# jbirky/alabi

Measured on AMD Instinct MI355X. Metric: surrogate_mcmc_samples_per_sec, higher is better.
Workload: dtype f64

## Files before the change

alabi_amd/_lib.py:

```python
from __future__ import annotations

import ctypes as C
import os
import subprocess

_HERE = os.path.dirname(os.path.abspath(__file__))
CSRC = os.path.join(_HERE, "csrc")
LIB_PATH = os.path.join(CSRC, "libalabi_hip.so")

OK, NOT_PD, BAD_ARG, HIP_ERROR, NOT_COMPUTED, TIMEOUT = 0, 1, 2, 3, 4, 5
UTILITY_CODES = {"bape": 0, "agp": 1, "jones": 2}
KERNEL_CODES = {"ExpSquaredKernel": 0, "Matern32Kernel": 1, "Matern52Kernel": 2, "RationalQuadraticKernel": 3}
MAX_DIM = 64

_vp, _i, _ll, _d = C.c_void_p, C.c_int, C.c_longlong, C.c_double
_ull = C.c_ulonglong
_pd = C.POINTER(C.c_double)
_pi = C.POINTER(C.c_int)
_pll = C.POINTER(C.c_longlong)

SIGNATURES = {
    "alabi_abi_version": (_i, []),
    "alabi_status_string": (C.c_char_p, [_i]),
    "alabi_last_error": (C.c_char_p, []),
# ... 29 lines not shown
    "alabi_kernel_matrix": (_i, [_vp, _i, _vp, _i, _i, _i, _d, _d, _pd, _vp, _vp]),
    "alabi_utility_scan": (_i, [_vp, _i, _vp, _ll, _pd, _d, _vp, _vp, _vp, _pd, _pll, _vp]),
    "alabi_utility_polish": (_i, [_vp, _i, _vp, _vp, _d, _i, _vp, _pd, _pi, _vp]),
    "alabi_utility_eval": (_i, [_i, _vp, _ll, _i, _pd, _d, _vp, _vp, _vp, _vp]),
    "alabi_ens_create": (_i, [_vp, _i, _i, _i, _pd, _ull, C.POINTER(_vp)]),
    "alabi_ens_destroy": (_i, [_vp]),
    "alabi_ens_set_logp_affine": (_i, [_vp, _d, _d]),
    "alabi_ens_set_normal_prior": (_i, [_vp, _pd, _pd]),
    "alabi_ens_set_logp_map": (_i, [_vp, _i]),
    "alabi_ens_surrogate": (_i, [_vp, _vp, _i, _vp, _vp]),
    "alabi_ens_propose": (_i, [_vp, _vp, _i, _i, _i, _vp, _vp, _vp]),
    "alabi_ens_accept": (_i, [_vp, _vp, _vp, _i, _i, _vp, _vp, _vp, _vp]),
    "alabi_ens_set_moves": (_i, [_vp, _i, _pi, _pd, _pd, _pd]),
    "alabi_ens_set_stream": (_i, [_vp, _i]),
    "alabi_ens_last_path": (_i, [_vp, _pi]),
    "alabi_ens_group_plan": (_i, [_vp, _pi]),
    "alabi_ens_lnprob": (_i, [_vp, _vp, _vp, _vp]),
    "alabi_ens_run": (_i, [_vp, _vp, _vp, _ll, _ll, _i, _d, _vp, _vp, _vp, _vp]),
    "alabi_chain_autocorr": (_i, [_vp, _ll, _i, _i, _vp, _vp]),
    "alabi_ens_draw": (_i, [_vp, _ll, _i, _d, _vp]),
    "alabi_ens_half_step": (_i, [_vp, _vp, _vp, _i, _i, _i, _i, _vp, _vp]),
    "alabi_dist_unique_id": (_i, [_vp]),
    "alabi_dist_comm_create": (_i, [_vp, _i, _i, C.POINTER(_vp)]),
    "alabi_dist_comm_create_callback": (_i, [_vp, _vp, _i, _i, C.POINTER(_vp)]),
    "alabi_dist_comm_destroy": (_i, [_vp]),
    "alabi_dist_comm_stats": (_i, [_vp, _pll]),
    "alabi_ens_run_sharded": (_i, [_vp, _vp, _vp, _vp, _ll, _ll, _i, _d, _vp, _vp, _vp, _vp]),
    "alabi_ens_step_lists": (_i, [_vp, _i, _vp, _pi, _vp]),
    "alabi_ens_step_with_randoms": (_i, [_vp, _vp, _vp, _vp, _i, _vp, _vp, _vp, _d, _vp, _vp]),
    "alabi_ens_export_draws": (_i, [_vp, _ll, _d, _vp, _pi, _vp, _vp, _vp, _vp, _vp, _vp]),
# ... 101 lines not shown
```

alabi_amd/csrc/api.hip:

```cpp
#include <atomic>
#include <cmath>
#include <cstdlib>
#include <mutex>
#include <new>
#include <vector>

#include "gp_device.hpp"

namespace alabi {
thread_local std::string g_last_error;

static inline hipStream_t as_stream(void* s) { return reinterpret_cast<hipStream_t>(s); }

__global__ void __launch_bounds__(256)
copy_factor_kernel(const double* __restrict__ L, int ld, int N, double* __restrict__ out) {
    size_t e = (size_t)blockIdx.x * 256 + threadIdx.x;
    if (e >= (size_t)N * N) return;
    int r = (int)(e / N), c = (int)(e % N);
    out[e] = (c <= r) ? L[(size_t)r * ld + c] : 0.0;
}

namespace {
struct CachedBuf { void* p; size_t bytes; };
std::mutex g_cache_mu;
// ... 560 lines not shown
int alabi_ens_destroy(alabi_ens* e) {
    if (!e) return ALABI_OK;
    if (e->graph_exec) (void)hipGraphExecDestroy(e->graph_exec);
    free_draws(e->draws);
    free_draws(e->draws2);
    free_move_buffers(e->mv);
    if (e->side_stream) (void)hipStreamDestroy(e->side_stream);
    if (e->ev_free) (void)hipEventDestroy(e->ev_free);
    if (e->ev_drawn) (void)hipEventDestroy(e->ev_drawn);
    if (e->run_state) (void)hipFree(e->run_state);
    if (e->consts) (void)hipFree(e->consts);
    if (e->hist) (void)hipFree(e->hist);
    if (e->part) (void)hipFree(e->part);
    if (e->cand) (void)hipFree(e->cand);
    if (e->err) (void)hipFree(e->err);
    delete e;
    return ALABI_OK;
}

int alabi_ens_set_normal_prior(alabi_ens* e, const double* mean, const double* std) {
    if (!e || !mean || !std) return ALABI_BAD_ARGUMENT;
    e->has_prior = 0; e->prior_const = 0.0;
    for (int k = 0; k < ALABI_MAX_DIM; ++k) { e->prior_mean[k] = 0.0; e->prior_istd[k] = 0.0; }
    for (int k = 0; k < e->d; ++k) {
        if (std::isfinite(mean[k]) && std::isfinite(std[k]) && std[k] > 0.0) {
            e->prior_mean[k] = mean[k];
            e->prior_istd[k] = 1.0 / std[k];
            e->prior_const += -std::log(std[k]) - 0.9189385332046727;
            e->has_prior = 1;
        }
// ... 38 lines not shown
    if (n > 0) { const int st = ensure_move_buffers(e); if (st != ALABI_OK) return st; }
    mt.n = n;
    e->moves = mt;
    e->has_de = de;
    e->drawn_n = 0;
    e->settings_gen++;
    if (e->graph_exec) { (void)hipGraphExecDestroy(e->graph_exec); e->graph_exec = nullptr; }
    return ALABI_OK;
}

int alabi_ens_set_stream(alabi_ens* e, int enabled) {
    if (!e) return ALABI_BAD_ARGUMENT;
    if (enabled && !(e->hist && e->err)) return ALABI_BAD_ARGUMENT;
    e->stream_ok = enabled ? 1 : 0;
    e->settings_gen++;
    return ALABI_OK;
}

int alabi_ens_last_path(alabi_ens* e, int* path) {
    if (!e || !path) return ALABI_BAD_ARGUMENT;
    *path = e->last_path;
    return ALABI_OK;
}

int alabi_ens_group_plan(alabi_ens* e, int* out) {
    if (!e || !out) return ALABI_BAD_ARGUMENT;
    for (int i = 0; i < 8; ++i) out[i] = e->group_plan[i];
    return ALABI_OK;
}

// ... 80 lines not shown
    hipStream_t s = as_stream(stream);
    int st;
    if ((st = sync_consts(e, s)) != ALABI_OK) return st;
    e->last_path = 0;
    const char* genv = getenv("ALABI_ENS_GROUP");
    const bool group_off = genv && genv[0] == '0', group_pref = genv && genv[0] == '1';
    const bool can_stream = ens_stream_fits(e);
    const bool crowded = can_stream && e->stream_grid > 0 && ((e->W + 1) / 2 + e->stream_grid - 1) / e->stream_grid >= 4;
    const bool use_group = !e->has_de && e->stream_ok && s != nullptr && !group_off && (group_pref || !can_stream || crowded) && ens_group_fits(e) &&
                           ens_group_buffers(e, s);
    if (!e->has_de && e->stream_ok && s != nullptr && (can_stream || use_group)) {
        e->last_path = use_group ? 3 : 1;
        const int need = (int)(nsteps < e->chunk_cap ? nsteps : e->chunk_cap);
        const int clean_rows = e->hist_clean;
        e->hist_clean = 0;
        if (use_group && (st = set_run_state(e, step0, 0, s)) != ALABI_OK) return st;
        ALABI_HIP_CHECK(hipMemsetAsync(e->err, 0, sizeof(int), s));
        long long remaining = nsteps;
        const bool two_sets = !use_group && nsteps > e->chunk_cap && ens_draw_ahead_ready(e);
        bool ahead_issued = false;
        while (remaining > 0) {
            const int K = (int)(remaining < e->chunk_cap ? remaining : e->chunk_cap);
            const long long done = nsteps - remaining;
            if (use_group) {
                if ((st = launch_ens_draw(e, K, a, s)) != ALABI_OK) return st;
                if ((st = launch_ens_group(e, coords, logp, K, thin_by, chain, chain_logp, n_accept, s)) != ALABI_OK) return st;
                if ((st = launch_ens_advance(e, K, s)) != ALABI_OK) return st;
            } else {
                const bool odd = two_sets && ((done / e->chunk_cap) & 1);
                const bool ahead = two_sets && remaining > K;
                const DrawBuffers& cur = odd ? e->draws2 : e->draws;
                if (ahead_issued) ALABI_HIP_CHECK(hipStreamWaitEvent(s, e->ev_drawn, 0));
                else if ((st = launch_ens_draw_at(e, cur, K, a, false, step0 + done, s)) != ALABI_OK) return st;
                ahead_issued = false;
                if (ahead) ALABI_HIP_CHECK(hipEventRecord(e->ev_free, s));
                if ((st = launch_ens_stream_kernel(e, cur, coords, logp, K, done == 0, (done == 0 && clean_rows < need) ? need : 0, s)) != ALABI_OK)
                    return st;
                if (ahead) {
                    const long long rem2 = remaining - K;
                    const int K2 = (int)(rem2 < e->chunk_cap ? rem2 : e->chunk_cap);
                    ALABI_HIP_CHECK(hipStreamWaitEvent(e->side_stream, e->ev_free, 0));
                    if ((st = launch_ens_draw_at(e, odd ? e->draws : e->draws2, K2, a, false, step0 + done + K, e->side_stream)) != ALABI_OK)
                        return st;
                    ALABI_HIP_CHECK(hipEventRecord(e->ev_drawn, e->side_stream));
                    ahead_issued = true;
                }
                if ((st = launch_ens_stream_epilogue(e, coords, logp, K, thin_by, chain, chain_logp, n_accept, step0 + done + K, done, s)) != ALABI_OK)
                    return st;
            }
            remaining -= K;
        }
        int flag = 0;
        ALABI_HIP_CHECK(hipMemcpyAsync(&flag, e->err, sizeof(int), hipMemcpyDeviceToHost, s));
        ALABI_HIP_CHECK(hipStreamSynchronize(s));
        e->hist_clean = (!use_group && !flag) ? (clean_rows > need ? clean_rows : need) : 0;
        return flag ? ALABI_TIMEOUT : ALABI_OK;
    }
    if ((st = set_run_state(e, step0, 0, s)) != ALABI_OK) return st;
    HalfArgs h = base_args(e, coords, logp);
    h.chain = chain; h.chain_logp = chain_logp; h.n_accept = n_accept; h.thin_by = thin_by;

    const char* env = getenv("ALABI_ENS_GRAPH");
    const bool want_graph = (s != nullptr) && !(env && env[0] == '0');
    int gsteps = e->chunk_cap < 256 ? e->chunk_cap : 256;
    if (const char* gs = getenv("ALABI_ENS_GRAPH_STEPS")) {
        int v = atoi(gs);
        if (v > 0 && v <= e->chunk_cap) gsteps = v;
    }
    long long remaining = nsteps;
    if (want_graph && remaining >= 2LL * gsteps) {
// ... 171 lines not shown
```

alabi_amd/csrc/common.hpp:

```cpp
#pragma once
#include <hip/hip_runtime.h>
#include <cstdint>
#include <cstdio>
#include <cstring>
#include <string>
#include <vector>

#include "../../include/alabi_hip.h"
#include "chol_tasks.hpp"

#define ALABI_BLK 64

namespace alabi {

extern thread_local std::string g_last_error;

inline int hip_fail(hipError_t e, const char* what, const char* file, int line) {
    char buf[512];
    snprintf(buf, sizeof(buf), "%s failed at %s:%d: %s", what, file, line, hipGetErrorString(e));
    g_last_error = buf;
    return ALABI_HIP_ERROR;
}

#define ALABI_HIP_CHECK(expr)                                                    \
// ... 122 lines not shown
        double a;
        long long gp_gen;
    } graph_key{};
    int graph_steps = 0;
    long long* run_state = nullptr;
    unsigned long long* hist = nullptr;
    int* err = nullptr;
    alabi::DrawBuffers draws2{};
    hipStream_t side_stream = nullptr;
    hipEvent_t ev_free = nullptr, ev_drawn = nullptr;
    int draws2_state = 0;
    int hist_clean = 0;
    int stream_grid = 0;
    int last_path = 0;
    int stream_ok = 0;
    unsigned long long* part = nullptr;
    size_t part_words = 0;
    unsigned long long* cand = nullptr;
    size_t cand_words = 0;
    long long settings_gen = 0;
    long long serial = 0;
    int group_plan[8] = {0};
    alabi::MoveTable moves{};
    bool has_de = false;
    alabi::MoveBuffers mv{};
};

namespace alabi {
int launch_prepare_inputs(alabi_gp* gp, const double* X, int N, hipStream_t s);
int launch_assemble(alabi_gp* gp, hipStream_t s, int zero_ctl_ints = 0);
// ... 71 lines not shown
int launch_ens_draw_at(alabi_ens* e, const DrawBuffers& into, int nsteps, double a, bool from_state, long long step0, hipStream_t s);
int launch_ens_prep(alabi_ens* e, const int* order, int n0, const double* u_z, const int* partner,
                    const double* u_acc, double a, hipStream_t s);
int launch_ens_prep_de(alabi_ens* e, const int* order, int n0, const int* j1, const int* j2, const double* gamma,
                       const double* u_acc, hipStream_t s);
int launch_ens_half_args(alabi_ens* e, const HalfArgs& args, int nblocks, hipStream_t s);
int launch_ens_lnprob(alabi_ens* e, const double* coords, int nwalkers, double* logp, int gate_box, hipStream_t s);
int launch_ens_propose(alabi_ens* e, const HalfArgs& args, int nblocks, int gate_box, double* q, double* like, hipStream_t s);
int launch_ens_accept(alabi_ens* e, const HalfArgs& args, int count, const double* q, const double* lp_new, hipStream_t s);
int launch_ens_advance(alabi_ens* e, long long n, hipStream_t s);
int ens_sync_consts(alabi_ens* e, hipStream_t s);
int alabi_ens_half_step_hist(alabi_ens* e, const double* coords, const double* logp, int t, int split, int part_begin, int part_end,
                             const double* shist, double* out, hipStream_t s);
bool ens_stream_fits(const alabi_ens* e);
int launch_ens_stream_kernel(alabi_ens* e, const DrawBuffers& rec, double* coords, double* logp, int K, bool first, int fill_rows, hipStream_t s);
int launch_ens_stream_epilogue(alabi_ens* e, double* coords, double* logp, int K, int thin_by, double* chain, double* chain_logp,
                               long long* n_accept, long long step_next, long long done0, hipStream_t s);
bool ens_group_fits(const alabi_ens* e);
bool ens_group_buffers(alabi_ens* e, hipStream_t s);
int launch_ens_group(alabi_ens* e, double* coords, double* logp, int K, int thin_by, double* chain, double* chain_logp,
                     long long* n_accept, hipStream_t s);
int launch_ens_hist_prologue(alabi_ens* e, double* coords, double* logp, int K, bool fill, hipStream_t s);
int launch_ens_hist_epilogue(alabi_ens* e, double* coords, double* logp, int K, int thin_by, double* chain, double* chain_logp,
                             long long* n_accept, hipStream_t s);
}
```

alabi_amd/csrc/ensemble.hip:

```cpp
#include <cstdlib>
#include <vector>
#include "ens_device.hpp"

namespace alabi {

__device__ inline void store_record(const DrawBuffers& b, size_t pos, int wid, int cw, double zz, double lnfac, double lnu) {
    b.order[pos] = wid;
    b.cw[pos] = cw;
    b.zz[pos] = zz;
    b.lnfac[pos] = lnfac;
    b.lnu[pos] = lnu;
    unsigned long long* pk = b.packed + 4 * pos;
    pk[0] = (unsigned long long)(unsigned)wid | ((unsigned long long)(unsigned)cw << 32);
    pk[1] = (unsigned long long)__double_as_longlong(zz);
    pk[2] = (unsigned long long)__double_as_longlong(lnfac);
    pk[3] = (unsigned long long)__double_as_longlong(lnu);
}

__device__ inline void write_record(const DrawBuffers& b, size_t pos, int wid, int cw, double u_z, double u_acc,
                                    double a, int d) {
    const double t1 = (a - 1.0) * u_z + 1.0;
    const double zz = (t1 * t1) / a;
    store_record(b, pos, wid, cw, zz, ((double)d - 1.0) * log(zz), log(u_acc));
}
// ... 565 lines not shown
    const int w = p.rec.order[pos];
    if (w < 0) return;
    const double lpn = lp_new[i], lpo = p.logp[w];
    if (p.rec.lnfac[pos] + lpn - lpo > p.rec.lnu[pos]) {
        for (int k = 0; k < p.d; ++k) p.coords[(size_t)w * p.d + k] = q[(size_t)i * p.d + k];
        p.logp[w] = lpn;
        if (p.n_accept) p.n_accept[w] += 1;
    }
}

__global__ void ens_advance_kernel(long long* run_state, long long n) {
    if (threadIdx.x == 0 && blockIdx.x == 0) { run_state[0] += n; run_state[1] += n; }
}


#define ALABI_HIST_EMPTY 0x7FF8A1AB1D15EA5Eull

struct StreamArgs {
    unsigned long long* hist;
    int* err;
    DrawBuffers rec;
    const double* consts;
    const double* Xt;
    const double* alpha;
    const double* centre;
    int K, W, n0, d, Npad, spin_limit, has_prior;
    double amp, mean, prior_const;
    KernelFn kf;
};

__device__ inline unsigned long long ld_sc1(const unsigned long long* p) {
    return __hip_atomic_load(p, __ATOMIC_RELAXED, __HIP_MEMORY_SCOPE_AGENT);
}
__device__ inline void st_sc1(unsigned long long* p, unsigned long long v) {
    __hip_atomic_store(p, v, __ATOMIC_RELAXED, __HIP_MEMORY_SCOPE_AGENT);
}

#ifdef ALABI_STREAM_PROF
__device__ long long g_stream_prof[16];
#endif

template <int NW>
__device__ inline double wave_partials_tree(const double* s) {
    const f64x2* v = reinterpret_cast<const f64x2*>(s);
    auto pair = [&](int i) { return 2 * i < NW ? v[i].y + v[i].x : 0.0; };
    const double lo8 = (pair(3) + pair(2)) + (pair(1) + pair(0));
    if (NW <= 8) return lo8;
    const double hi8 = (pair(7) + pair(6)) + (pair(5) + pair(4));
    return hi8 + lo8;
}

template <int D, int PPT, int TMAX, bool GENERIC>
__global__ void __launch_bounds__(TMAX)
ens_stream_kernel(StreamArgs p) {
    __shared__ __attribute__((aligned(16))) double scratch[2][16];
    __shared__ unsigned long long rec_s[4][4];
    __shared__ __attribute__((aligned(16))) double qs_s[2][ALABI_MAX_DIM];
    __shared__ double consts_s[6][ALABI_MAX_DIM];
    __shared__ int abort_s;
    static_assert(D < ALABI_MAX_DIM && TMAX >= 192 && TMAX % 64 == 0, "ens_stream_kernel: shape");
    constexpr int TC = TMAX - 128, nwc = TC >> 6;
    const int tid = threadIdx.x, lane = tid & 63;
    const int wv = __builtin_amdgcn_readfirstlane(tid >> 6);
    const bool comm = wv == 0, service = wv == nwc + 1, compute = !comm && !service;
    const int b = blockIdx.x, e = blockIdx.y, E = gridDim.y;
// ... 351 lines not shown
    return ALABI_OK;
}

int launch_ens_hist_epilogue(alabi_ens* e, double* coords, double* logp, int K, int thin_by, double* chain, double* chain_logp,
                             long long* n_accept, hipStream_t s) {
    const int WT = e->W * e->E, row = e->d + 2;
    hipLaunchKernelGGL(ens_hist_copy_kernel, dim3((WT * row + 255) / 256), dim3(256), 0, s, coords, logp,
                       e->hist + (size_t)K * WT * row, WT, e->d, 0);
    if (chain || chain_logp || n_accept)
        hipLaunchKernelGGL(ens_hist_chain_kernel, dim3(2048), dim3(256), 0, s, e->hist, K, WT, e->d, thin_by, e->run_state,
                           e->err, chain, chain_logp, reinterpret_cast<unsigned long long*>(n_accept));
    ALABI_LAUNCH_CHECK();
    return ALABI_OK;
}

int launch_ens_stream_kernel(alabi_ens* e, const DrawBuffers& rec, double* coords, double* logp, int K, bool first, int fill_rows,
                             hipStream_t s) {
    alabi_gp* gp = e->gp;
    const int n0 = (e->W + 1) / 2;
    const int WT = e->W * e->E, row = e->d + 2;
    if (fill_rows > 0) hipLaunchKernelGGL(ens_hist_fill_kernel, dim3(1024), dim3(256), 0, s, e->hist + (size_t)WT * row, (size_t)fill_rows * WT * row);
    if (first) hipLaunchKernelGGL(ens_hist_copy_kernel, dim3((WT * row + 255) / 256), dim3(256), 0, s, coords, logp, e->hist, WT, e->d, 1);
    StreamArgs a{};
    a.hist = e->hist; a.err = e->err; a.rec = rec; a.consts = e->consts;
    const bool se = gp->kf.type == 0;
    a.Xt = se ? gp->Xc : gp->Xt; a.alpha = se ? gp->ens_h : gp->alpha; a.centre = gp->xa_centre;
    a.K = K; a.W = e->W; a.n0 = n0; a.d = e->d; a.Npad = gp->Npad; a.spin_limit = 1 << 20;
    if (const char* env = getenv("ALABI_ENS_SPIN_LIMIT")) { const int v = atoi(env); if (v > 0) a.spin_limit = v; }
    a.amp = e->lp_scale * exp(gp->log_amp); a.mean = fma(e->lp_scale, gp->mean, e->lp_shift); a.kf = gp->kf;
    a.has_prior = e->has_prior; a.prior_const = e->prior_const;
    const int db = dim_bucket(e->d);
    const int T = e->threads, ppt = ens_stream_ppt(e);
    e->last_path = 1;
    if (T == 256) {
        if (ppt == 1) { ALABI_STREAM_LAUNCH(1, 384); }
        else if (ppt == 2) { ALABI_STREAM_LAUNCH(2, 384); }
        else if (ppt == 3) { ALABI_STREAM_LAUNCH(3, 384); }
        else if (ppt == 4) { ALABI_STREAM_LAUNCH(4, 384); }
        else return ALABI_BAD_ARGUMENT;
    } else if (T == 512) {
        if (ppt == 1) { ALABI_STREAM_LAUNCH(1, 640); }
        else if (ppt == 2) { ALABI_STREAM_LAUNCH(2, 640); }
        else return ALABI_BAD_ARGUMENT;
    } else return ALABI_BAD_ARGUMENT;
    ALABI_LAUNCH_CHECK();
// ... 137 lines not shown
```

alabi_amd/sampler.py:

```python
from __future__ import annotations

import ctypes as C
import time

import numpy as np
import torch

from . import _lib
from .gp import HipGP, _dev, _to_dev
from .mcmc_utils import integrated_time
from .moves import parse_moves

__all__ = ["EnsembleSampler", "State"]


class State:
    def __init__(self, coords, log_prob=None):
        self.coords = coords
        self.log_prob = log_prob
        self.blobs = None
        self.random_state = None

    def __iter__(self):
        return iter((self.coords, self.log_prob, self.random_state))
# ... 268 lines not shown
                                                nsteps, thin_by, self.a, _lib.ptr(chain), _lib.ptr(chain_lp),
                                                _lib.ptr(self._naccept), C.c_void_p(self._stream.cuda_stream))

        st = _run()
        if st == _lib.TIMEOUT:
            self._stream.synchronize()
            self._coords.copy_(backup[0]); self._logp.copy_(backup[1]); self._naccept.copy_(backup[2])
            _lib.check(_lib.lib().alabi_ens_set_stream(self._ens, 0), "alabi_ens_set_stream")
            self.stream_fallbacks = getattr(self, "stream_fallbacks", 0) + 1
            st = _run()
        _lib.check(st, "alabi_ens_run")
        path = C.c_int(0)
        _lib.lib().alabi_ens_last_path(self._ens, C.byref(path))
        self.last_path = {1: "stream", 3: "group"}.get(path.value, "launch-per-half-step")
        self.last_stream_kernel = {1: "ens_stream_kernel", 3: "ens_group_kernel"}.get(path.value)
        self.group_plan = None
        if path.value == 3:
            plan = (C.c_int * 8)()
            _lib.lib().alabi_ens_group_plan(self._ens, plan)
            self.group_plan = dict(zip(("Q", "G", "NG", "RT", "tpm", "ltw", "KS", "lds_bytes"), (int(v) for v in plan)))
        self._stream.synchronize()
        torch.cuda.current_stream().wait_stream(self._stream)
        self.last_run_seconds = time.perf_counter() - t0
        self.iteration += nsteps
        self._rng_step += nsteps
        if nstore:
            self._chains.append(chain)
            self._chain_lps.append(chain_lp)
            self._thins.append(thin_by)
        return State(self._coords.cpu().numpy(), self._logp.cpu().numpy())
# ... 42 lines not shown
```

include/alabi_hip.h:

```cpp
#ifndef ALABI_HIP_H
#define ALABI_HIP_H

#ifdef __cplusplus
extern "C" {
#endif

#define ALABI_OK 0
#define ALABI_NOT_POSITIVE_DEFINITE 1
#define ALABI_BAD_ARGUMENT 2
#define ALABI_HIP_ERROR 3
#define ALABI_NOT_COMPUTED 4
#define ALABI_TIMEOUT 5

#define ALABI_UTILITY_BAPE 0
#define ALABI_UTILITY_AGP 1
#define ALABI_UTILITY_JONES 2

#define ALABI_MAX_DIM 64

typedef struct alabi_gp alabi_gp;
typedef struct alabi_ens alabi_ens;
typedef struct alabi_ns alabi_ns;
typedef struct alabi_kde alabi_kde;

// ... 67 lines not shown
                       void* stream);

int alabi_ens_create(alabi_gp* gp, int W, int d, int n_ensembles, const double* bounds,
                     unsigned long long seed, alabi_ens** out);
int alabi_ens_destroy(alabi_ens* ens);
int alabi_ens_set_normal_prior(alabi_ens* ens, const double* mean, const double* std);

int alabi_ens_set_logp_affine(alabi_ens* ens, double scale, double shift);

int alabi_ens_set_logp_map(alabi_ens* ens, int kind);

int alabi_ens_set_moves(alabi_ens* ens, int n, const int* kind, const double* cum, const double* p0, const double* p1);

int alabi_ens_set_stream(alabi_ens* ens, int enabled);
int alabi_ens_last_path(alabi_ens* ens, int* path );
int alabi_ens_group_plan(alabi_ens* ens, int* out );

int alabi_ens_lnprob(alabi_ens* ens, const double* coords, double* logp, void* stream);

int alabi_ens_surrogate(alabi_ens* ens, const double* points, int M, double* like, void* stream);

int alabi_ens_run(alabi_ens* ens, double* coords, double* logp, long long step0,
                  long long nsteps, int thin_by, double a, double* chain, double* chain_logp,
                  long long* n_accept, void* stream);

int alabi_chain_autocorr(const double* chain, long long n_t, int n_w, int n_d, double* acf_mean, void* stream);

int alabi_ens_draw(alabi_ens* ens, long long step0, int nsteps, double a, void* stream);
int alabi_ens_half_step(alabi_ens* ens, double* coords, double* logp, int t, int split,
                        int part_begin, int part_end, long long* n_accept, void* stream);
// ... 77 lines not shown
```

Before: 84.76 million.

## Add paired-block speculative stream kernel for ensemble MCMC sampling

Adds a new ens_pair_kernel variant of the persistent stream kernel in which each walker item is handled by two cooperating blocks. One block speculatively evaluates the surrogate on a proposal built from not-yet-final coordinates and publishes it to a separate proposal history buffer, which shortens the dependency chain between half-steps. The run loop selects the pair variant when the group path is not used and the extra buffers can be allocated. It saves coords, logp and accept counts first so that a timeout can roll back and re-run on the single-block path. This costs twice the blocks, extra history memory and fill traffic, and adds spin-wait and correctness risk.

```diff
diff --git a/alabi_amd/_lib.py b/alabi_amd/_lib.py
--- a/alabi_amd/_lib.py
+++ b/alabi_amd/_lib.py
@@ -67,6 +67,8 @@
     "alabi_ens_set_moves": (_i, [_vp, _i, _pi, _pd, _pd, _pd]),
     "alabi_ens_set_stream": (_i, [_vp, _i]),
     "alabi_ens_last_path": (_i, [_vp, _pi]),
+    "alabi_ens_stream_variant": (_i, [_vp, _pi]),
+    "alabi_ens_pair_stats": (_i, [_vp, _pll, _i]),
     "alabi_ens_group_plan": (_i, [_vp, _pi]),
     "alabi_ens_lnprob": (_i, [_vp, _vp, _vp, _vp]),
     "alabi_ens_run": (_i, [_vp, _vp, _vp, _ll, _ll, _i, _d, _vp, _vp, _vp, _vp]),
diff --git a/alabi_amd/csrc/api.hip b/alabi_amd/csrc/api.hip
--- a/alabi_amd/csrc/api.hip
+++ b/alabi_amd/csrc/api.hip
@@ -598,6 +598,7 @@
     if (e->part) (void)hipFree(e->part);
     if (e->cand) (void)hipFree(e->cand);
     if (e->err) (void)hipFree(e->err);
+    ens_pair_release(e);
     delete e;
     return ALABI_OK;
 }
@@ -666,6 +667,24 @@
     if (enabled && !(e->hist && e->err)) return ALABI_BAD_ARGUMENT;
     e->stream_ok = enabled ? 1 : 0;
     e->settings_gen++;
+    return ALABI_OK;
+}
+
+int alabi_ens_stream_variant(alabi_ens* e, int* variant) {
+    if (!e || !variant) return ALABI_BAD_ARGUMENT;
+    *variant = (e->last_path == 1) ? e->last_variant : 0;
+    return ALABI_OK;
+}
+
+int alabi_ens_pair_stats(alabi_ens* e, long long* out, int reset) {
+    if (!e || !out) return ALABI_BAD_ARGUMENT;
+    if (!e->pair_stats) {
+        ALABI_HIP_CHECK(hipMalloc(&e->pair_stats, 9 * sizeof(unsigned long long)));
+        ALABI_HIP_CHECK(hipMemset(e->pair_stats, 0, 9 * sizeof(unsigned long long)));
+    }
+    ALABI_HIP_CHECK(hipDeviceSynchronize());
+    ALABI_HIP_CHECK(hipMemcpy(out, e->pair_stats, 9 * sizeof(unsigned long long), hipMemcpyDeviceToHost));
+    if (reset) ALABI_HIP_CHECK(hipMemset(e->pair_stats, 0, 9 * sizeof(unsigned long long)));
     return ALABI_OK;
 }
 
@@ -776,6 +795,15 @@
         const int need = (int)(nsteps < e->chunk_cap ? nsteps : e->chunk_cap);
         const int clean_rows = e->hist_clean;
         e->hist_clean = 0;
+        const bool use_pair = !use_group && can_stream && ens_pair_ready(e);
+        e->last_variant = use_pair ? 1 : 0;
+        const size_t WTs = (size_t)e->W * e->E;
+        if (use_pair) {
+            double* sv = e->pair_save;
+            ALABI_HIP_CHECK(hipMemcpyAsync(sv, coords, WTs * e->d * sizeof(double), hipMemcpyDeviceToDevice, s));
+            ALABI_HIP_CHECK(hipMemcpyAsync(sv + WTs * e->d, logp, WTs * sizeof(double), hipMemcpyDeviceToDevice, s));
+            if (n_accept) ALABI_HIP_CHECK(hipMemcpyAsync(sv + WTs * (e->d + 1), n_accept, WTs * sizeof(long long), hipMemcpyDeviceToDevice, s));
+        }
         if (use_group && (st = set_run_state(e, step0, 0, s)) != ALABI_OK) return st;
         ALABI_HIP_CHECK(hipMemsetAsync(e->err, 0, sizeof(int), s));
         long long remaining = nsteps;
@@ -796,7 +824,9 @@
                 else if ((st = launch_ens_draw_at(e, cur, K, a, false, step0 + done, s)) != ALABI_OK) return st;
                 ahead_issued = false;
                 if (ahead) ALABI_HIP_CHECK(hipEventRecord(e->ev_free, s));
-                if ((st = launch_ens_stream_kernel(e, cur, coords, logp, K, done == 0, (done == 0 && clean_rows < need) ? need : 0, s)) != ALABI_OK)
+                const int fill_rows = (done == 0 && clean_rows < need) ? need : 0;
+                if ((st = use_pair ? launch_ens_pair_kernel(e, cur, coords, logp, K, done == 0, fill_rows, s)
+                                   : launch_ens_stream_kernel(e, cur, coords, logp, K, done == 0, fill_rows, s)) != ALABI_OK)
                     return st;
                 if (ahead) {
                     const long long rem2 = remaining - K;
@@ -816,6 +846,14 @@
         ALABI_HIP_CHECK(hipMemcpyAsync(&flag, e->err, sizeof(int), hipMemcpyDeviceToHost, s));
         ALABI_HIP_CHECK(hipStreamSynchronize(s));
         e->hist_clean = (!use_group && !flag) ? (clean_rows > need ? clean_rows : need) : 0;
+        if (flag && use_pair) {
+            const double* sv = e->pair_save;
+            ALABI_HIP_CHECK(hipMemcpyAsync(coords, sv, WTs * e->d * sizeof(double), hipMemcpyDeviceToDevice, s));
+            ALABI_HIP_CHECK(hipMemcpyAsync(logp, sv + WTs * e->d, WTs * sizeof(double), hipMemcpyDeviceToDevice, s));
+            if (n_accept) ALABI_HIP_CHECK(hipMemcpyAsync(n_accept, sv + WTs * (e->d + 1), WTs * sizeof(long long), hipMemcpyDeviceToDevice, s));
+            e->pair_state = -1;
+            return alabi_ens_run(e, coords, logp, step0, nsteps, thin_by, a, chain, chain_logp, n_accept, stream);
+        }
         return flag ? ALABI_TIMEOUT : ALABI_OK;
     }
     if ((st = set_run_state(e, step0, 0, s)) != ALABI_OK) return st;
diff --git a/alabi_amd/csrc/common.hpp b/alabi_amd/csrc/common.hpp
--- a/alabi_amd/csrc/common.hpp
+++ b/alabi_amd/csrc/common.hpp
@@ -160,6 +160,11 @@
     int stream_grid = 0;
     int last_path = 0;
     int stream_ok = 0;
+    unsigned long long* prop = nullptr;
+    double* pair_save = nullptr;
+    unsigned long long* pair_stats = nullptr;
+    int pair_state = 0;
+    int last_variant = 0;
     unsigned long long* part = nullptr;
     size_t part_words = 0;
     unsigned long long* cand = nullptr;
@@ -261,6 +266,12 @@
                              const double* shist, double* out, hipStream_t s);
 bool ens_stream_fits(const alabi_ens* e);
 int launch_ens_stream_kernel(alabi_ens* e, const DrawBuffers& rec, double* coords, double* logp, int K, bool first, int fill_rows, hipStream_t s);
+int ens_stream_ppt_of(const alabi_ens* e);
+int launch_ens_hist_fill(unsigned long long* rows, size_t words, hipStream_t s);
+int launch_ens_stream_prologue(alabi_ens* e, double* coords, double* logp, bool first, int fill_rows, hipStream_t s);
+bool ens_pair_ready(alabi_ens* e);
+void ens_pair_release(alabi_ens* e);
+int launch_ens_pair_kernel(alabi_ens* e, const DrawBuffers& rec, double* coords, double* logp, int K, bool first, int fill_rows, hipStream_t s);
 int launch_ens_stream_epilogue(alabi_ens* e, double* coords, double* logp, int K, int thin_by, double* chain, double* chain_logp,
                                long long* n_accept, long long step_next, long long done0, hipStream_t s);
 bool ens_group_fits(const alabi_ens* e);
diff --git a/alabi_amd/csrc/ens_pair.hip b/alabi_amd/csrc/ens_pair.hip
--- /dev/null
+++ b/alabi_amd/csrc/ens_pair.hip
@@ -0,0 +1,430 @@
+#include <cstdlib>
+#include "ens_stream.hpp"
+
+namespace alabi {
+
+struct PairArgs {
+    StreamArgs s;
+    unsigned long long* prop;
+    unsigned long long* stats;
+};
+
+#ifdef ALABI_PAIR_PROF
+__device__ long long g_pair_prof[24];
+#define ALABI_PAIR_PUB_MASK ((1 << 19) - 1)
+__device__ long long g_pair_pub[2][ALABI_PAIR_PUB_MASK + 1];
+__device__ inline void pair_pub_stamp(int which, size_t row_index) {
+    __hip_atomic_store(&g_pair_pub[which][row_index & ALABI_PAIR_PUB_MASK], wall_clock64(), __ATOMIC_RELAXED, __HIP_MEMORY_SCOPE_AGENT);
+}
+__device__ inline long long pair_pub_age(int which, size_t row_index, long long now) {
+    const long long dt = now - __hip_atomic_load(&g_pair_pub[which][row_index & ALABI_PAIR_PUB_MASK], __ATOMIC_RELAXED, __HIP_MEMORY_SCOPE_AGENT);
+    return (dt > 0 && dt < 100000) ? dt : -1;
+}
+#endif
+
+template <int D, int PPT, int TMAX, bool GENERIC>
+__global__ void __launch_bounds__(TMAX)
+ens_pair_kernel(PairArgs pa) {
+    const StreamArgs& p = pa.s;
+    __shared__ __attribute__((aligned(16))) double scratch[2][16];
+    __shared__ unsigned long long rec_s[4][6];
+    __shared__ __attribute__((aligned(16))) double qs_s[2][ALABI_MAX_DIM];
+    __shared__ double consts_s[6][ALABI_MAX_DIM];
+    __shared__ int abort_s;
+    static_assert(D < ALABI_MAX_DIM && TMAX >= 192 && TMAX % 64 == 0, "ens_pair_kernel: shape");
+    constexpr int TC = TMAX - 128, nwc = TC >> 6;
+    const int tid = threadIdx.x, lane = tid & 63;
+    const int wv = __builtin_amdgcn_readfirstlane(tid >> 6);
+    const bool comm = wv == 0, service = wv == nwc + 1, compute = !comm && !service;
+    const int b = blockIdx.x >> 1, e = blockIdx.y, E = gridDim.y;
+    const int role_a = blockIdx.x & 1;
+    const int WT = p.W * E, row = p.d + 2;
+#ifdef ALABI_PAIR_PROF
+    long long prof[11] = {0, 0, 0, 0, 0, 0, 0, 0, 0, 0, 0};
+    const long long prof_begin = wall_clock64();
+#endif
+    const int half = p.Npad >> 1, ct = tid - 64;
+    f64x2 xa[PPT][D], aa[PPT];
+#pragma unroll
+    for (int j = 0; j < PPT; ++j) {
+        const int idx = ct + j * TC;
+        const bool v = compute && idx < half;
+#pragma unroll
+        for (int k = 0; k < D; ++k)
+            xa[j][k] = v ? reinterpret_cast<const f64x2*>(p.Xt + (size_t)k * p.Npad)[idx] : f64x2{0.0, 0.0};
+        aa[j] = v ? reinterpret_cast<const f64x2*>(p.alpha)[idx] : (GENERIC ? f64x2{0.0, 0.0} : f64x2{ALABI_SE_PAD, ALABI_SE_PAD});
+    }
+    if (tid < ALABI_MAX_DIM) {
+        consts_s[0][tid] = (tid < p.d) ? p.consts[tid] : 0.0;
+        consts_s[1][tid] = (tid < p.d) ? p.consts[ALABI_MAX_DIM + tid] : 0.0;
+        consts_s[2][tid] = (tid < p.d) ? p.consts[2 * ALABI_MAX_DIM + tid] : 0.0;
+        consts_s[3][tid] = (tid < p.d) ? p.consts[3 * ALABI_MAX_DIM + tid] : 0.0;
+        consts_s[4][tid] = (tid < p.d) ? p.consts[4 * ALABI_MAX_DIM + tid] : 0.0;
+        consts_s[5][tid] = (!GENERIC && tid < p.d) ? p.centre[tid] : 0.0;
+    }
+    if (tid < 32) scratch[tid >> 4][tid & 15] = 0.0;
+    if (tid == 0) abort_s = 0;
+
+    const int G = gridDim.x >> 1;
+    auto next_item = [&](int& t, int& split, int& bb) {
+        bb += G;
+        for (;;) {
+            if (t >= p.K) return;
+            if (bb < (split ? p.W - p.n0 : p.n0)) return;
+            bb = b;
+            if (split == 0) split = 1; else { split = 0; ++t; }
+        }
+    };
+    const unsigned long long* packed = p.rec.packed;
+    const int* pos_of = p.rec.pos_of;
+    auto record_load = [&](int t, int split, int bb) -> unsigned long long {
+        if (t >= p.K || lane >= 4) return 0ull;
+        const size_t pos = ((size_t)t * E + e) * p.W + (split ? p.n0 : 0) + bb;
+        return packed[4 * pos + lane];
+    };
+    auto fresh_load = [&](int t, int split, unsigned long long rec) -> unsigned long long {
+        const int w = __builtin_amdgcn_readlane((int)(unsigned)(rec & 0xffffffffull), 0);
+        const int cw = __builtin_amdgcn_readlane((int)(unsigned)(rec >> 32), 0);
+        if (t >= p.K || (lane != 4 && lane != 5)) return 0ull;
+        if (split) return lane == 5 ? 1ull : 0ull;
+        if (t == 0) return 0ull;
+        return pos_of[(size_t)(t - 1) * WT + (lane == 4 ? w : cw)] >= p.n0 ? 1ull : 0ull;
+    };
+    unsigned long long rec_a = 0, fresh_a = 0, rec_b = 0;
+    int bt = 0, bsplit = 0;
+    int pt = 0, psplit = 0, pbb = b, pslot = 0;
+    if (service) {
+        for (int i = 0; i < 2; ++i) {
+            const unsigned long long r = record_load(pt, psplit, pbb);
+            const unsigned long long f = fresh_load(pt, psplit, r);
+            if (lane < 6) rec_s[pslot & 3][lane] = lane < 4 ? r : f;
+            next_item(pt, psplit, pbb); ++pslot;
+        }
+        rec_a = record_load(pt, psplit, pbb);
+        fresh_a = fresh_load(pt, psplit, rec_a);
+        next_item(pt, psplit, pbb);
+        bt = pt; bsplit = psplit;
+        rec_b = record_load(pt, psplit, pbb);
+        next_item(pt, psplit, pbb);
+    }
+    __syncthreads();
+    int t = 0, split = 0, bb = b, item = 0;
+
+    if (comm) {
+        const int n0_lane = lane < p.d ? lane : p.d, n1_lane = lane < p.d ? lane : p.d - 1;
+        const int out_lane = lane <= p.d ? lane : p.d + 1, ver_lane = lane == p.d ? p.d : p.d + 1;
+        const long long prop_off = (long long)(pa.prop - p.hist);
+        int n_mode = 0, n_own_a = 0;
+        double n_zz = 0.0;
+        size_t n_out = 0;
+#ifdef ALABI_PAIR_PROF
+        size_t n_fidx = 0;
+#endif
+        int n_cls = 0;
+        const unsigned long long *n_hw = p.hist, *n_hc = p.hist, *n_ver = p.hist;
+        auto decode_next = [&](int it, int tt, int sp) {
+            const unsigned long long* rs = rec_s[it & 3];
+            const unsigned long long ids = rs[0];
+            const int w = (int)(unsigned)(ids & 0xffffffffull);
+            const int cw = (int)(unsigned)(ids >> 32);
+            n_zz = __longlong_as_double((long long)rs[1]);
+            n_cls = (int)rs[4] + (int)rs[5];
+            const int fo = __builtin_amdgcn_readfirstlane((int)rs[4]), fp = __builtin_amdgcn_readfirstlane((int)rs[5]);
+            const int spec = (fo + fp) == 1;
+            n_mode = spec ? 1 : role_a ? 2 : 0;
+            n_own_a = spec & role_a & fo;
+            const int vo = tt, vp = tt + sp;
+            const int rv_o = vo - (spec & !role_a & fo), rv_p = vp - (spec & !role_a & fp);
+            const size_t row_o = ((size_t)rv_o * WT + w) * row, row_p = ((size_t)rv_p * WT + cw) * row;
+            const bool prop_o = spec && role_a && fo, prop_p = spec && role_a && fp;
+            n_hw = p.hist + (row_o + (prop_o ? n1_lane : n0_lane)) + (prop_o ? prop_off : 0ll);
+            n_hc = p.hist + (row_p + n1_lane) + (prop_p ? prop_off : 0ll);
+            if (n_mode == 2) { n_hw = p.hist + n0_lane; n_hc = p.hist + n1_lane; }
+            n_ver = p.hist + ((size_t)(fo ? vo : vp) * WT + (fo ? w : cw)) * row + ver_lane;
+            n_out = ((size_t)(tt + 1) * WT + w) * row + out_lane;
+#ifdef ALABI_PAIR_PROF
+            n_fidx = (size_t)(fo ? vo : vp) * WT + (fo ? w : cw);
+#endif
+        };
+        const double il_r = consts_s[0][lane], lo_r = consts_s[1][lane], hi_r = consts_s[2][lane], c_r = consts_s[5][lane];
+        const bool needc = lane < p.d;
+        const unsigned long long coord_lanes = (1ull << p.d) - 1;
+        int st_items = 0, st_rows = 0;
+        decode_next(0, 0, 0);
+        while (t < p.K) {
+            const int par = item & 1;
+#ifdef ALABI_PAIR_PROF
+            const long long c0 = wall_clock64();
+#endif
+            unsigned long long ws, wc;
+            int spins = 0;
+            bool pending;
+            for (;;) {
+                ws = ld_sc1(n_hw);
+                wc = ld_sc1(n_hc);
+                pending = __builtin_amdgcn_ballot_w64(ws == ALABI_HIST_EMPTY || wc == ALABI_HIST_EMPTY) != 0;
+                if (!pending) break;
+                if (__builtin_expect(++spins > p.spin_limit || ((spins & 63) == 0 && __builtin_amdgcn_readfirstlane(
+                        __hip_atomic_load(p.err, __ATOMIC_RELAXED, __HIP_MEMORY_SCOPE_AGENT)) != 0), 0)) break;
+            }
+            if (__builtin_expect(pending, 0)) {
+                n_zz = __builtin_nan("");
+                abort_s = 1;
+                __hip_atomic_store(p.err, 1, __ATOMIC_RELAXED, __HIP_MEMORY_SCOPE_AGENT);
+            }
+#ifdef ALABI_PAIR_PROF
+            const long long c1 = wall_clock64();
+            const size_t fidx = n_fidx;
+            if (n_mode == 1 && role_a && !pending) { const long long dt = pair_pub_age(0, fidx, c1); if (dt > 0) { prof[7] += dt; prof[8] += 1; } }
+#endif
+            const int mode = n_mode, own_a = n_own_a, cls = n_cls;
+            const size_t out_word = n_out;
+            const unsigned long long* ver = n_ver;
+            const double sv = __longlong_as_double((long long)ws), cv = __longlong_as_double((long long)wc);
+            const double qv = cv - (cv - sv) * n_zz;
+            const bool all_in = mode != 2 && (__builtin_amdgcn_ballot_w64(qv > lo_r) & __builtin_amdgcn_ballot_w64(qv < hi_r) & coord_lanes)
+                                                 == coord_lanes;
+            double qs = qv * il_r;
+            if (!GENERIC) qs -= c_r;
+            qs_s[par][lane] = needc ? qs : 0.0;
+            reinterpret_cast<int*>(&qs_s[par][D])[1] = all_in ? 0x3ff00000 : 0;
+#ifdef ALABI_PAIR_PROF
+            if (mode == 0 && !pending) pair_pub_stamp(0, out_word / row);
+#endif
+            if (mode == 0 && !pending) st_sc1(p.hist + (out_word + prop_off), (unsigned long long)__double_as_longlong(qv));
+            __syncthreads();
+            __builtin_amdgcn_sched_barrier(0);
+#ifdef ALABI_PAIR_PROF
+            const long long c2 = wall_clock64();
+#endif
+            int t2 = t, s2 = split, b2 = bb;
+            next_item(t2, s2, b2);
+            if (pending) t2 = p.K;
+            double prior_q = 0.0;
+            if (p.has_prior) {
+                const double u = (qv - consts_s[3][lane]) * consts_s[4][lane];
+                prior_q = lane_bcast(wave_sum_dpp(needc ? -0.5 * u * u : 0.0), 63) + p.prior_const;
+            }
+            double lnfac = __longlong_as_double((long long)rec_s[item & 3][2]);
+            double lnu = __longlong_as_double((long long)rec_s[item & 3][3]);
+            double lp_old = lane_bcast(sv, p.d);
+            int part = par * (int)sizeof(scratch[0]);
+            if (t2 < p.K) decode_next(item + 1, t2, s2);
+            int win = mode == 0;
+#ifdef ALABI_PAIR_PROF
+            const long long c2v = wall_clock64();
+#endif
+            if (mode == 1 && !pending) {
+                unsigned long long vw;
+                bool vpend;
+                int vspins = 0;
+                for (;;) {
+                    vw = ld_sc1(ver);
+                    vpend = __builtin_amdgcn_ballot_w64(vw == ALABI_HIST_EMPTY) != 0;
+                    if (!vpend) break;
+                    if (__builtin_expect(++vspins > p.spin_limit || ((vspins & 63) == 0 && __builtin_amdgcn_readfirstlane(
+                            __hip_atomic_load(p.err, __ATOMIC_RELAXED, __HIP_MEMORY_SCOPE_AGENT)) != 0), 0)) break;
+                }
+                if (__builtin_expect(vpend, 0)) {
+                    abort_s = 1;
+                    __hip_atomic_store(p.err, 1, __ATOMIC_RELAXED, __HIP_MEMORY_SCOPE_AGENT);
+                    t2 = p.K;
+                }
+                const int flag = __builtin_amdgcn_readfirstlane((int)(unsigned)(vw & 0xffffffffull));
+                win = !vpend && flag == role_a;
+#ifdef ALABI_PAIR_PROF
+                if (win) pair_pub_stamp(0, out_word / row);
+#endif
+                if (win) st_sc1(p.hist + (out_word + prop_off), (unsigned long long)__double_as_longlong(qv));
+                if (own_a) lp_old = lane_bcast(__longlong_as_double((long long)vw), p.d);
+            }
+#ifdef ALABI_PAIR_PROF
+            const long long c2w = wall_clock64();
+            if (mode == 1 && !pending) { const long long dt = pair_pub_age(1, fidx, c2w); if (dt > 0) { prof[9] += dt; prof[10] += 1; } }
+#endif
+            unsigned long long w_rej = needc ? ws : lane == p.d ? (unsigned long long)__double_as_longlong(lp_old) : 0ull;
+            unsigned long long w_acc = !all_in ? w_rej : needc ? (unsigned long long)__double_as_longlong(qv) : 1ull;
+            const bool takes_lp = all_in && lane == p.d;
+            if (pending) win = 0;
+            if (pa.stats) { st_items += (cls == lane); st_rows += (cls == lane && win); }
+            size_t ow = out_word;
+            asm volatile("" : "+v"(ow), "+v"(w_rej), "+v"(w_acc), "+v"(lp_old), "+v"(lnfac), "+v"(lnu), "+v"(prior_q), "+v"(part));
+            __builtin_amdgcn_sched_barrier(0);
+            __syncthreads();
+#ifdef ALABI_PAIR_PROF
+            const long long c3 = wall_clock64();
+#endif
+            const double* partials = reinterpret_cast<const double*>(reinterpret_cast<const char*>(&scratch[0][0]) + part);
+            const double lp_new = fma(p.amp, wave_partials_tree<nwc>(partials), p.mean) + prior_q;
+            const bool acc = lnfac + lp_new - lp_old > lnu;
+            if (takes_lp) w_acc = (unsigned long long)__double_as_longlong(lp_new);
+#ifdef ALABI_PAIR_PROF
+            if (win) pair_pub_stamp(1, ow / row);
+#endif
+            if (win) st_sc1(p.hist + ow, acc ? w_acc : w_rej);
+            t = t2; split = s2; bb = b2; ++item;
+#ifdef ALABI_PAIR_PROF
+            { const long long c4 = wall_clock64();
+              prof[0] += c1 - c0; prof[1] += c2 - c1; prof[2] += c3 - c2; prof[3] += c4 - c3; prof[4] += 1;
+              if (mode == 1) { prof[5] += c2w - c2v; prof[6] += 1; } }
+#endif
+        }
+        if (pa.stats && lane < 3) {
+            if (!role_a) atomicAdd(pa.stats + 3 * lane, (unsigned long long)st_items);
+            atomicAdd(pa.stats + 3 * lane + 1 + role_a, (unsigned long long)st_rows);
+        }
+#ifdef ALABI_PAIR_PROF
+        if (tid == 0 && b == 3 && blockIdx.y == 0) {
+            long long* g = g_pair_prof + 8 * role_a;
+            for (int i = 0; i < 5; ++i) g[i] = prof[i];
+            g[5] = wall_clock64() - prof_begin;
+            g[6] = prof[5]; g[7] = prof[6];
+            for (int i = 0; i < 4; ++i) g_pair_prof[16 + 4 * role_a + i] = prof[7 + i];
+        }
+#endif
+    } else if (compute) {
+        while (t < p.K) {
+            next_item(t, split, bb);
+            const int par = item & 1;
+            __syncthreads();
+            double q[D];
+#pragma unroll
+            for (int k = 0; k < D; ++k) {
+                const double r = qs_s[par][k];
+                q[k] = __hiloint2double(__builtin_amdgcn_readfirstlane(__double2hiint(r)),
+                                        __builtin_amdgcn_readfirstlane(__double2loint(r)));
+            }
+            const int inb = __builtin_amdgcn_readfirstlane(__double2hiint(qs_s[par][D]));
+            __builtin_amdgcn_sched_group_barrier(0x100, D + 1, 0);
+            __builtin_amdgcn_sched_group_barrier(0x2, 2 * D + 1, 0);
+            if (inb != 0) {
+                double acc = 0.0;
+                if (!GENERIC) {
+                    const double nhq = se_neg_half_norm<D>(q);
+#pragma unroll
+                    for (int j = 0; j < PPT; ++j) {
+                        double fa, fb;
+                        se_pair_terms<D>(xa[j], aa[j], q, nhq, fa, fb);
+                        acc += fa; acc += fb;
+                        if ((j & 1) == 1) __builtin_amdgcn_sched_barrier(0);
+                    }
+                } else
+#pragma unroll
+                for (int j = 0; j < PPT; ++j) {
+                    double r2a = 0.0, r2b = 0.0;
+#pragma unroll
+                    for (int k = 0; k < D; ++k) {
+                        const double da = xa[j][k].x - q[k], db = xa[j][k].y - q[k];
+                        r2a = fma(da, da, r2a);
+                        r2b = fma(db, db, r2b);
+                    }
+                    acc = (j == 0) ? aa[j].x * radial<GENERIC>(r2a, p.kf) : fma(aa[j].x, radial<GENERIC>(r2a, p.kf), acc);
+                    acc = fma(aa[j].y, radial<GENERIC>(r2b, p.kf), acc);
+                    if ((j & 1) == 1) __builtin_amdgcn_sched_barrier(0);
+                }
+                const double wsum = wave_sum_dpp(acc);
+                if (lane == 63) scratch[par][wv - 1] = wsum;
+            }
+            __syncthreads();
+            if (abort_s) return;
+            ++item;
+        }
+    } else {
+        while (t < p.K) {
+            next_item(t, split, bb);
+            __syncthreads();
+            if (lane < 6) rec_s[pslot & 3][lane] = lane < 4 ? rec_a : fresh_a;
+            ++pslot;
+            rec_a = rec_b;
+            fresh_a = fresh_load(bt, bsplit, rec_a);
+            bt = pt; bsplit = psplit;
+            rec_b = record_load(pt, psplit, pbb);
+            next_item(pt, psplit, pbb);
+            __syncthreads();
+            if (abort_s) return;
+        }
+    }
+}
+
+#ifdef ALABI_PAIR_PROF
+extern "C" int alabi_debug_pair_prof(long long* out) {
+    return (int)hipMemcpyFromSymbol(out, HIP_SYMBOL(g_pair_prof), sizeof(long long) * 24);
+}
+#endif
+
+#define ALABI_PAIR_DISPATCH_DIM(DB, ...)                              \
+    switch (DB) {                                                     \
+        case 1: { constexpr int D = 1; __VA_ARGS__; } break;          \
+        case 2: { constexpr int D = 2; __VA_ARGS__; } break;          \
+        case 3: { constexpr int D = 3; __VA_ARGS__; } break;          \
+        case 4: { constexpr int D = 4; __VA_ARGS__; } break;          \
+        case 5: { constexpr int D = 5; __VA_ARGS__; } break;          \
+        case 6: { constexpr int D = 6; __VA_ARGS__; } break;          \
+        case 8: { constexpr int D = 8; __VA_ARGS__; } break;          \
+        case 10: { constexpr int D = 10; __VA_ARGS__; } break;        \
+        case 12: { constexpr int D = 12; __VA_ARGS__; } break;        \
+        case 16: { constexpr int D = 16; __VA_ARGS__; } break;        \
+        default: return ALABI_BAD_ARGUMENT;                           \
+    }
+#define ALABI_PAIR_LAUNCH(PPT_, TMAX_)                                                                            \
+    ALABI_PAIR_DISPATCH_DIM(db, ALABI_DISPATCH_KERNEL(gp->kf.type,                                                \
+        hipLaunchKernelGGL((ens_pair_kernel<D, PPT_, TMAX_, GENERIC>), dim3(2 * n0, e->E), dim3(TMAX_), 0, s, a)))
+
+bool ens_pair_ready(alabi_ens* e) {
+    if (e->pair_state < 0) return false;
+    if (e->pair_state == 0) {
+        e->pair_state = -1;
+        const char* env = getenv("ALABI_ENS_PAIR");
+        if (env && env[0] == '0') return false;
+        int dev = 0, n_cu = 0;
+        if (hipGetDevice(&dev) != hipSuccess || hipDeviceGetAttribute(&n_cu, hipDeviceAttributeMultiprocessorCount, dev) != hipSuccess) return false;
+        const long long wgs = 2LL * ((e->W + 1) / 2) * e->E;
+        if (e->d < 1 || wgs > n_cu) return false;
+        const size_t WT = (size_t)e->W * e->E, row = e->d + 2;
+        const size_t words = ((size_t)e->chunk_cap + 1) * WT * row;
+        if (hipMalloc(&e->prop, words * sizeof(unsigned long long)) != hipSuccess) { (void)hipGetLastError(); e->prop = nullptr; return false; }
+        if (hipMalloc(&e->pair_save, (WT * (e->d + 1)) * sizeof(double) + WT * sizeof(long long)) != hipSuccess) {
+            (void)hipGetLastError(); (void)hipFree(e->prop); e->prop = nullptr; e->pair_save = nullptr; return false;
+        }
+        e->pair_state = 1;
+    }
+    return true;
+}
+
+void ens_pair_release(alabi_ens* e) {
+    if (e->prop) (void)hipFree(e->prop);
+    if (e->pair_save) (void)hipFree(e->pair_save);
+    if (e->pair_stats) (void)hipFree(e->pair_stats);
+    e->prop = nullptr; e->pair_save = nullptr; e->pair_stats = nullptr;
+}
+
+int launch_ens_pair_kernel(alabi_ens* e, const DrawBuffers& rec, double* coords, double* logp, int K, bool first, int fill_rows,
+                           hipStream_t s) {
+    alabi_gp* gp = e->gp;
+    const int n0 = (e->W + 1) / 2;
+    const int WT = e->W * e->E, row = e->d + 2;
+    int st = launch_ens_stream_prologue(e, coords, logp, first, fill_rows, s);
+    if (st != ALABI_OK) return st;
+    if ((st = launch_ens_hist_fill(e->prop + (size_t)WT * row, (size_t)K * WT * row, s)) != ALABI_OK) return st;
+    PairArgs a{};
+    a.s = ens_stream_args(e, rec, K);
+    a.prop = e->prop; a.stats = e->pair_stats;
+    const int db = dim_bucket(e->d);
+    const int T = e->threads, ppt = ens_stream_ppt_of(e);
+    e->last_path = 1;
+    if (T == 256) {
+        if (ppt == 1) { ALABI_PAIR_LAUNCH(1, 384); }
+        else if (ppt == 2) { ALABI_PAIR_LAUNCH(2, 384); }
+        else if (ppt == 3) { ALABI_PAIR_LAUNCH(3, 384); }
+        else if (ppt == 4) { ALABI_PAIR_LAUNCH(4, 384); }
+        else return ALABI_BAD_ARGUMENT;
+    } else if (T == 512) {
+        if (ppt == 1) { ALABI_PAIR_LAUNCH(1, 640); }
+        else if (ppt == 2) { ALABI_PAIR_LAUNCH(2, 640); }
+        else return ALABI_BAD_ARGUMENT;
+    } else return ALABI_BAD_ARGUMENT;
+    ALABI_LAUNCH_CHECK();
+    return ALABI_OK;
+}
+
+}
diff --git a/alabi_amd/csrc/ens_stream.hpp b/alabi_amd/csrc/ens_stream.hpp
--- /dev/null
+++ b/alabi_amd/csrc/ens_stream.hpp
@@ -0,0 +1,40 @@
+#pragma once
+#include "ens_device.hpp"
+
+namespace alabi {
+
+#define ALABI_HIST_EMPTY 0x7FF8A1AB1D15EA5Eull
+
+struct StreamArgs {
+    unsigned long long* hist;
+    int* err;
+    DrawBuffers rec;
+    const double* consts;
+    const double* Xt;
+    const double* alpha;
+    const double* centre;
+    int K, W, n0, d, Npad, spin_limit, has_prior;
+    double amp, mean, prior_const;
+    KernelFn kf;
+};
+
+StreamArgs ens_stream_args(alabi_ens* e, const DrawBuffers& rec, int K);
+
+__device__ inline unsigned long long ld_sc1(const unsigned long long* p) {
+    return __hip_atomic_load(p, __ATOMIC_RELAXED, __HIP_MEMORY_SCOPE_AGENT);
+}
+__device__ inline void st_sc1(unsigned long long* p, unsigned long long v) {
+    __hip_atomic_store(p, v, __ATOMIC_RELAXED, __HIP_MEMORY_SCOPE_AGENT);
+}
+
+template <int NW>
+__device__ inline double wave_partials_tree(const double* s) {
+    const f64x2* v = reinterpret_cast<const f64x2*>(s);
+    auto pair = [&](int i) { return 2 * i < NW ? v[i].y + v[i].x : 0.0; };
+    const double lo8 = (pair(3) + pair(2)) + (pair(1) + pair(0));
+    if (NW <= 8) return lo8;
+    const double hi8 = (pair(7) + pair(6)) + (pair(5) + pair(4));
+    return hi8 + lo8;
+}
+
+}
diff --git a/alabi_amd/csrc/ensemble.hip b/alabi_amd/csrc/ensemble.hip
--- a/alabi_amd/csrc/ensemble.hip
+++ b/alabi_amd/csrc/ensemble.hip
@@ -1,6 +1,6 @@
 #include <cstdlib>
 #include <vector>
-#include "ens_device.hpp"
+#include "ens_stream.hpp"
 
 namespace alabi {
 
@@ -603,41 +603,9 @@
 }
 
 
-#define ALABI_HIST_EMPTY 0x7FF8A1AB1D15EA5Eull
-
-struct StreamArgs {
-    unsigned long long* hist;
-    int* err;
-    DrawBuffers rec;
-    const double* consts;
-    const double* Xt;
-    const double* alpha;
-    const double* centre;
-    int K, W, n0, d, Npad, spin_limit, has_prior;
-    double amp, mean, prior_const;
-    KernelFn kf;
-};
-
-__device__ inline unsigned long long ld_sc1(const unsigned long long* p) {
-    return __hip_atomic_load(p, __ATOMIC_RELAXED, __HIP_MEMORY_SCOPE_AGENT);
-}
-__device__ inline void st_sc1(unsigned long long* p, unsigned long long v) {
-    __hip_atomic_store(p, v, __ATOMIC_RELAXED, __HIP_MEMORY_SCOPE_AGENT);
-}
-
 #ifdef ALABI_STREAM_PROF
 __device__ long long g_stream_prof[16];
 #endif
-
-template <int NW>
-__device__ inline double wave_partials_tree(const double* s) {
-    const f64x2* v = reinterpret_cast<const f64x2*>(s);
-    auto pair = [&](int i) { return 2 * i < NW ? v[i].y + v[i].x : 0.0; };
-    const double lo8 = (pair(3) + pair(2)) + (pair(1) + pair(0));
-    if (NW <= 8) return lo8;
-    const double hi8 = (pair(7) + pair(6)) + (pair(5) + pair(4));
-    return hi8 + lo8;
-}
 
 template <int D, int PPT, int TMAX, bool GENERIC>
 __global__ void __launch_bounds__(TMAX)
@@ -1019,21 +987,41 @@
     return ALABI_OK;
 }
 
-int launch_ens_stream_kernel(alabi_ens* e, const DrawBuffers& rec, double* coords, double* logp, int K, bool first, int fill_rows,
-                             hipStream_t s) {
-    alabi_gp* gp = e->gp;
-    const int n0 = (e->W + 1) / 2;
+int ens_stream_ppt_of(const alabi_ens* e) { return ens_stream_ppt(e); }
+
+int launch_ens_hist_fill(unsigned long long* rows, size_t words, hipStream_t s) {
+    hipLaunchKernelGGL(ens_hist_fill_kernel, dim3(1024), dim3(256), 0, s, rows, words);
+    ALABI_LAUNCH_CHECK();
+    return ALABI_OK;
+}
+
+int launch_ens_stream_prologue(alabi_ens* e, double* coords, double* logp, bool first, int fill_rows, hipStream_t s) {
     const int WT = e->W * e->E, row = e->d + 2;
     if (fill_rows > 0) hipLaunchKernelGGL(ens_hist_fill_kernel, dim3(1024), dim3(256), 0, s, e->hist + (size_t)WT * row, (size_t)fill_rows * WT * row);
     if (first) hipLaunchKernelGGL(ens_hist_copy_kernel, dim3((WT * row + 255) / 256), dim3(256), 0, s, coords, logp, e->hist, WT, e->d, 1);
+    ALABI_LAUNCH_CHECK();
+    return ALABI_OK;
+}
+
+StreamArgs ens_stream_args(alabi_ens* e, const DrawBuffers& rec, int K) {
+    alabi_gp* gp = e->gp;
     StreamArgs a{};
     a.hist = e->hist; a.err = e->err; a.rec = rec; a.consts = e->consts;
     const bool se = gp->kf.type == 0;
     a.Xt = se ? gp->Xc : gp->Xt; a.alpha = se ? gp->ens_h : gp->alpha; a.centre = gp->xa_centre;
-    a.K = K; a.W = e->W; a.n0 = n0; a.d = e->d; a.Npad = gp->Npad; a.spin_limit = 1 << 20;
+    a.K = K; a.W = e->W; a.n0 = (e->W + 1) / 2; a.d = e->d; a.Npad = gp->Npad; a.spin_limit = 1 << 20;
     if (const char* env = getenv("ALABI_ENS_SPIN_LIMIT")) { const int v = atoi(env); if (v > 0) a.spin_limit = v; }
     a.amp = e->lp_scale * exp(gp->log_amp); a.mean = fma(e->lp_scale, gp->mean, e->lp_shift); a.kf = gp->kf;
     a.has_prior = e->has_prior; a.prior_const = e->prior_const;
+    return a;
+}
+
+int launch_ens_stream_kernel(alabi_ens* e, const DrawBuffers& rec, double* coords, double* logp, int K, bool first, int fill_rows,
+                             hipStream_t s) {
+    alabi_gp* gp = e->gp;
+    int st = launch_ens_stream_prologue(e, coords, logp, first, fill_rows, s);
+    if (st != ALABI_OK) return st;
+    const StreamArgs a = ens_stream_args(e, rec, K);
     const int db = dim_bucket(e->d);
     const int T = e->threads, ppt = ens_stream_ppt(e);
     e->last_path = 1;
diff --git a/alabi_amd/sampler.py b/alabi_amd/sampler.py
--- a/alabi_amd/sampler.py
+++ b/alabi_amd/sampler.py
@@ -306,6 +306,9 @@
         _lib.lib().alabi_ens_last_path(self._ens, C.byref(path))
         self.last_path = {1: "stream", 3: "group"}.get(path.value, "launch-per-half-step")
         self.last_stream_kernel = {1: "ens_stream_kernel", 3: "ens_group_kernel"}.get(path.value)
+        variant = C.c_int(0)
+        _lib.lib().alabi_ens_stream_variant(self._ens, C.byref(variant))
+        self.last_stream_variant = {0: "single", 1: "pair"}[variant.value] if path.value == 1 else None
         self.group_plan = None
         if path.value == 3:
             plan = (C.c_int * 8)()
diff --git a/include/alabi_hip.h b/include/alabi_hip.h
--- a/include/alabi_hip.h
+++ b/include/alabi_hip.h
@@ -105,6 +105,8 @@
 
 int alabi_ens_set_stream(alabi_ens* ens, int enabled);
 int alabi_ens_last_path(alabi_ens* ens, int* path );
+int alabi_ens_stream_variant(alabi_ens* ens, int* variant );
+int alabi_ens_pair_stats(alabi_ens* ens, long long* out , int reset);
 int alabi_ens_group_plan(alabi_ens* ens, int* out );
 
 int alabi_ens_lnprob(alabi_ens* ens, const double* coords, double* logp, void* stream);
```

Result: faster. 90.72 million, median of 6 (+7.0%).
